# arkworks-rs/groth16

Hardware: AMD Instinct MI355X
Metric: R1CS constraints/sec (create_proof, BLS12-381) (higher is better)
Workload: dtype u32-limb Montgomery integers (Fr 255-bit, Fq 381-bit); 1 GPU; SYN(k=22) synthetic R1CS, 4194302 constraints, FFT domain 2^22, bls12_381, full create_proof (7 NTTs + 4 G1 MSMs + 1 G2 MSM), valid proving key generated on the GPU from seeded toxic waste; curve=bls12_381, log2_domain=22, constraints=4194302, key=valid, witness=resident in HBM at entry (--full: value_incl_h2d holds the PCIe-inclusive rates), parallelism=single-gpu

## Files before the change

groth16_amd/csrc/internal.hpp:

```cpp
#pragma once
#include <hip/hip_runtime.h>
#include <atomic>
#include <cstdint>
#include <cstdio>
#include <cstring>
#include <string>
#include <vector>
#include "../../include/g16_mi355x.h"
#include "curve.hpp"

namespace g16 {

void set_last_error(const char* what, hipError_t e, const char* file, int line);

#define G16_HIP_TRY(expr)                                                     \
    do {                                                                      \
        hipError_t e__ = (expr);                                              \
        if (e__ != hipSuccess) {                                              \
            ::g16::set_last_error(#expr, e__, __FILE__, __LINE__);            \
            return e__ == hipErrorOutOfMemory ? G16_ERR_OOM : G16_ERR_HIP;    \
        }                                                                     \
    } while (0)

#define G16_TRY(expr)                  \
// ... 73 lines not shown
                                    const typename C::Fr* cst, hipStream_t st);
template <class C> int scale_by_table(typename C::Fr* data, const typename C::Fr* table, size_t n, hipStream_t st);
template <class C> int gen_power_table(typename C::Fr* out, size_t n, const typename C::Fr& base, const typename C::Fr& scale, bool r30_form,
                                       hipStream_t st);

template <class C>
struct DeviceCircuit {
    typedef typename C::Fr Fr;
    uint64_t num_inputs = 0, num_constraints = 0, num_variables = 0;
    uint64_t* row_ptr[3] = {nullptr, nullptr, nullptr};
    uint32_t* col[3] = {nullptr, nullptr, nullptr};
    Fr* val[3] = {nullptr, nullptr, nullptr};
    uint64_t nnz[3] = {0, 0, 0};
    Domain<C>* dom = nullptr;
    static constexpr int Z_CHUNKS = 8;
    uint64_t need_col[Z_CHUNKS] = {};
};
struct ZUpload {
    const void* host = nullptr;
    hipStream_t copy_stream = nullptr;
    hipEvent_t landed[8] = {};
    int pieces = 0;
};
template <class C> int mark_unit_coefficients(DeviceCircuit<C>* ck, hipStream_t st);
template <class C> int witness_map_device(const DeviceCircuit<C>* ck, const typename C::Fr* d_z, typename C::Fr* d_h, Arena& arena,
                                          hipStream_t st, EventTimer* ntt_timers = nullptr, ZUpload* up = nullptr);

template <class C>
struct DistWm {
    typedef typename C::Fr Fr;
    int rank = 0, world = 1, log_world = 0;
    size_t M = 0, blk = 0;
    Domain<C>* dom_m = nullptr;
    Fr* tw1 = nullptr;
    Fr* sc_mid = nullptr;
    Fr* tw2 = nullptr;
    Fr* sc_out = nullptr;
    Fr wn_fwd[8], wn_inv[8];
    Fr zinv;
};
template <class C> int dwm_create(const DeviceCircuit<C>* ck, int rank, int world, hipStream_t st, DistWm<C>** out);
template <class C> void dwm_destroy(DistWm<C>* d);
template <class C> int dwm_stage(const DeviceCircuit<C>* ck, const DistWm<C>* dw, int stage, const typename C::Fr* d_z,
                                 typename C::Fr* const work[3], typename C::Fr* const recv[3], typename C::Fr* h_local, hipStream_t st);

struct MsmPlan {
    int c = 0;
    int W = 0;
    int groups = 0;
    bool merged = false;
    uint32_t B = 0;
    uint32_t Lmax = 0;
    int affine_levels = 0;
    uint32_t chunk = 0;
    uint32_t K[10];
    int shard_n = 1, shard_r = 0;
    uint32_t buckets() const { return B * (uint32_t)groups; }
    uint32_t G = 8;
    uint32_t chunk_buckets() const { return B >= G ? G : B; }
    uint32_t chunks() const { return B / chunk_buckets(); }
    int chunk_bits() const { int k = 0; while ((1u << k) < chunks()) ++k; return k; }
    int planes() const { return 2 + chunk_bits(); }
    int outputs() const { return groups * planes(); }
};
static constexpr int MSM_MAX_OUTPUTS = 256;
static constexpr int MSM_MERGED_MIN_C = 9, MSM_MERGED_MAX_C = 20;
static constexpr uint64_t MSM_MERGED_MAX_N = (uint64_t)1 << 26;
int make_msm_plan(uint64_t n, int scalar_bits, const uint32_t* modulus_words, int mod_nwords, int merged_c, MsmPlan* plan, int shard_n = 1,
                  int shard_r = 0);
int msm_window_override();
int merged_window_bits(uint64_t n, int scalar_bits, const uint32_t* modulus_words, int mod_nwords);
int msm_plan_windows(int c, int scalar_bits, const uint32_t* modulus_words, int mod_nwords);

struct ScalarSort {
    MsmPlan plan;
    uint64_t n = 0;
    uint32_t* sorted = nullptr;
    uint32_t* offsets = nullptr;
    uint32_t* task_off = nullptr;
    uint32_t* heavy = nullptr;
    uint32_t max_tasks = 0;
    uint32_t max_segments = 0;
    uint64_t max_sorted = 0;
};
template <class C> int sort_scalars(const typename C::Fr* d_scalars, uint64_t n, int merged_c, Arena& arena, hipStream_t st, ScalarSort* out,
                                    int shard_n = 1, int shard_r = 0);

template <class F>
struct MsmBuffers {
    void* partials = nullptr;
    void* chunk_out = nullptr;
    XYZZ<F>* window_sums = nullptr;
};
template <class F> int msm_bucket_pass(const Affine<F>* d_bases, int64_t shift, uint64_t base_count, const ScalarSort& ss, Arena& arena,
                                       hipStream_t st, MsmBuffers<F>* out, EventTimer* bucket_timer);
template <class F>
struct PassJob {
    const Affine<F>* bases;
    int64_t shift;
    uint64_t base_count;
    const ScalarSort* ss;
    MsmBuffers<F>* out;
};
template <class F> int msm_bucket_pass_batch(const PassJob<F>* jobs, int n, Arena& arena, hipStream_t st, EventTimer* bucket_timer);
template <class F> int msm_reduce(const MsmBuffers<F>& buf, const ScalarSort& ss, hipStream_t st);
template <class F> int msm_reduce_batch(const MsmBuffers<F>* const* bufs, const ScalarSort* const* sorts, int n, hipStream_t st, bool heavy_done);
template <class F> int msm_heavy_reduce(const MsmBuffers<F>& buf, const ScalarSort& ss, hipStream_t st);
template <class F> int msm_heavy_reduce_batch(const MsmBuffers<F>* const* bufs, const ScalarSort* const* sorts, int n, hipStream_t st);
template <class F> int convert_bases(Affine<F>* d_bases, uint64_t n, hipStream_t st);
template <class F> XYZZ<F> fold_windows(const XYZZ<F>* window_sums, const MsmPlan& plan);
template <class F> int build_window_tables(const Affine<F>* d_src, uint64_t n, int c, int W, Affine<F>* d_table, hipStream_t st, void* park = nullptr);
template <class F> size_t window_table_park_bytes(uint64_t n, int W);

template <class C>
int generate_parameters_device(hipStream_t st, Arena& arena, const g16_csr_view abc[3], uint64_t ni, uint64_t nc, uint64_t nv,
                               const g16_toxic_waste* tw, const uint64_t* g1_gen, const uint64_t* g2_gen, const g16_params_view* out);
template <class C>
int qap_evaluations_host(const g16_csr_view abc[3], uint64_t ni, uint64_t nc, uint64_t nv, const uint64_t* t, uint64_t* a_out, uint64_t* b_out,
                         uint64_t* c_out, uint64_t* zt_out);

int serialize_points(int curve, int g2, int compressed, const uint64_t* points, uint64_t n, uint8_t* out);
int deserialize_points(int curve, int g2, int compressed, const uint8_t* in, uint64_t n, int validate, uint64_t* points_out);
uint64_t serialized_point_size(int curve, int g2, int compressed);

int mad_rate_device(hipStream_t st, double* mad_per_s);
template <class C> int synth_bases_device(int g2, uint64_t seed, uint64_t first, uint64_t n, void* out_dev, hipStream_t st);

}
```

groth16_amd/csrc/msm.hip:

```cpp
#include "internal.hpp"
#include "msm_common.hpp"
#include "fp30.hpp"
#include "batch_affine.hpp"
#include "window_tables.hpp"
#include <algorithm>
#include <cstdlib>

namespace g16 {

static constexpr int SORT_THREADS = 1024;
static constexpr int ACC_THREADS = 64;
static constexpr int RED_THREADS = 64;
static constexpr int WIN_THREADS = 256;
#ifndef G16_REDUCE_G
#define G16_REDUCE_G 8
#endif
static constexpr uint32_t REDUCE_G = G16_REDUCE_G;

struct PlanDev {
    int c, W;
    uint32_t B;
    uint32_t K[10];
    uint32_t shard_n, shard_r, shard_magic;
};
// ... 34 lines not shown
    uint32_t* hist = reinterpret_cast<uint32_t*>(smem);
    const int w = blockIdx.y;
    for (uint32_t b = threadIdx.x; b < B; b += SORT_THREADS) hist[b] = 0;
    __syncthreads();
    const uint64_t lo = (uint64_t)blockIdx.x * chunk, hi = min(n, lo + chunk);
    const uint16_t* plane = planes + (uint64_t)w * n;
    for (uint64_t p = lo + threadIdx.x; p < hi; p += SORT_THREADS) {
        uint32_t bucket, neg;
        if (digit_to_bucket(plane[p], c, &bucket, &neg)) atomicAdd(&hist[bucket], 1u);
    }
    __syncthreads();
    uint32_t* out = counts + (uint64_t)w * B;
    for (uint32_t b = threadIdx.x; b < B; b += SORT_THREADS) {
        const uint32_t v = hist[b];
        if (v) atomicAdd(&out[b], v);
    }
}

static constexpr int CLASS_THREADS = 256;
static constexpr int MAX_CLASSES = 64;
static constexpr uint32_t SORT_CLASS_LOG = 13;
static constexpr int SORT_M_THREADS = 256;

template <class Fr>
__device__ __forceinline__ void biased_scalar(const Fr& sc, const PlanDev& plan, uint32_t (*sw)[CLASS_THREADS]) {
    uint32_t s[Fr::N];
    sc.to_canonical(s);
    uint64_t carry = 0;
    G16_UNROLL for (int k = 0; k < 10; ++k) {
        carry += (uint64_t)(k < Fr::N ? s[k] : 0u) + plan.K[k];
        sw[k][threadIdx.x] = (uint32_t)carry;
        carry >>= 32;
    }
    sw[10][threadIdx.x] = 0;
}
__device__ __forceinline__ uint32_t window_of(const uint32_t (*sw)[CLASS_THREADS], int w, int c) {
    const int bit = w * c, word = bit >> 5, sh = bit & 31;
    const uint64_t two = (uint64_t)sw[word][threadIdx.x] | ((uint64_t)sw[word + 1][threadIdx.x] << 32);
    return (uint32_t)(two >> sh) & ((1u << c) - 1u);
}

template <class Fr>
__global__ __launch_bounds__(CLASS_THREADS) void class_count_kernel(const Fr* __restrict__ scalars, uint64_t n, PlanDev plan, uint32_t blog,
                                                                    uint32_t Q, uint32_t* __restrict__ block_counts) {
    __shared__ uint32_t sw[MSM_SWORDS][CLASS_THREADS];
    __shared__ uint32_t cnt[MAX_CLASSES];
    if (threadIdx.x < MAX_CLASSES) cnt[threadIdx.x] = 0;
    __syncthreads();
    const uint64_t i = (uint64_t)blockIdx.x * CLASS_THREADS + threadIdx.x;
    if (i < n) {
        biased_scalar(scalars[i], plan, sw);
        for (int w = 0; w < plan.W; ++w) {
            uint32_t key, neg;
            if (digit_to_bucket(window_of(sw, w, plan.c), plan.c, &key, &neg) && shard_local_key(plan, &key)) atomicAdd(&cnt[key >> blog], 1u);
        }
    }
    __syncthreads();
    if (threadIdx.x < Q) block_counts[(uint64_t)threadIdx.x * gridDim.x + blockIdx.x] = cnt[threadIdx.x];
}

template <class Fr>
__global__ __launch_bounds__(CLASS_THREADS) void class_partition_kernel(const Fr* __restrict__ scalars, uint64_t n, PlanDev plan, uint32_t blog,
                                                                        uint32_t Q, const uint32_t* __restrict__ block_off,
                                                                        uint16_t* __restrict__ ent_key, uint32_t* __restrict__ ent_tag) {
    __shared__ uint32_t sw[MSM_SWORDS][CLASS_THREADS];
    __shared__ uint32_t cur[MAX_CLASSES];
    if (threadIdx.x < Q) cur[threadIdx.x] = block_off[(uint64_t)threadIdx.x * gridDim.x + blockIdx.x];
    __syncthreads();
    const uint64_t i = (uint64_t)blockIdx.x * CLASS_THREADS + threadIdx.x;
    if (i >= n) return;
    biased_scalar(scalars[i], plan, sw);
    for (int w = 0; w < plan.W; ++w) {
        uint32_t key, neg;
        if (digit_to_bucket(window_of(sw, w, plan.c), plan.c, &key, &neg) && shard_local_key(plan, &key)) {
            const uint32_t pos = atomicAdd(&cur[key >> blog], 1u);
            ent_key[pos] = (uint16_t)((key & ((1u << blog) - 1u)) | (neg << 15));
            ent_tag[pos] = (uint32_t)i | ((uint32_t)w << 26);
        }
    }
}

static __global__ __launch_bounds__(SORT_M_THREADS) void bucket_count_merged_kernel(const uint16_t* __restrict__ ent_key,
                                                                           const uint32_t* __restrict__ class_off, uint32_t nb, uint32_t B,
                                                                           uint32_t* __restrict__ wg_counts) {
    extern __shared__ __attribute__((aligned(16))) unsigned char smem[];
    uint32_t* hist = reinterpret_cast<uint32_t*>(smem);
    const uint32_t q = blockIdx.y;
    const uint32_t lo = class_off[(uint64_t)q * nb], hi = class_off[(uint64_t)(q + 1) * nb];
    for (uint32_t b = threadIdx.x; b < B; b += SORT_M_THREADS) hist[b] = 0;
    __syncthreads();
    for (uint64_t p = (uint64_t)lo + blockIdx.x * SORT_M_THREADS + threadIdx.x; p < hi; p += (uint64_t)gridDim.x * SORT_M_THREADS)
        atomicAdd(&hist[ent_key[p] & 0x7fffu], 1u);
    __syncthreads();
    uint32_t* out = wg_counts + ((uint64_t)q * gridDim.x + blockIdx.x) * B;
    for (uint32_t b = threadIdx.x; b < B; b += SORT_M_THREADS) out[b] = hist[b];
}

static __global__ __launch_bounds__(256) void bucket_wg_scan_kernel(uint32_t* __restrict__ wg_counts, uint32_t G, uint32_t B, uint32_t M,
                                                                    uint32_t* __restrict__ counts) {
    const uint32_t i = blockIdx.x * 256 + threadIdx.x;
    if (i >= M) return;
    const uint32_t q = i / B, b = i - q * B;
    uint32_t* col = wg_counts + (uint64_t)q * G * B + b;
    uint32_t run = 0;
    for (uint32_t x = 0; x < G; ++x) {
        const uint32_t v = col[(uint64_t)x * B];
        col[(uint64_t)x * B] = run;
        run += v;
    }
    counts[i] = run;
}

static __global__ __launch_bounds__(SORT_M_THREADS) void bucket_scatter_merged_kernel(const uint16_t* __restrict__ ent_key,
                                                                             const uint32_t* __restrict__ ent_tag,
                                                                             const uint32_t* __restrict__ class_off, uint32_t nb, uint32_t B,
                                                                             const uint32_t* __restrict__ offsets,
                                                                             const uint32_t* __restrict__ wg_counts, uint32_t* __restrict__ sorted) {
    extern __shared__ __attribute__((aligned(16))) unsigned char smem[];
    uint32_t* hist = reinterpret_cast<uint32_t*>(smem);
    const uint32_t q = blockIdx.y;
    const uint32_t lo = class_off[(uint64_t)q * nb], hi = class_off[(uint64_t)(q + 1) * nb];
    if ((uint64_t)lo + (uint64_t)blockIdx.x * SORT_M_THREADS >= hi) return;
    const uint64_t qb = (uint64_t)q * B;
    const uint32_t* mine = wg_counts + ((uint64_t)q * gridDim.x + blockIdx.x) * B;
    for (uint32_t b = threadIdx.x; b < B; b += SORT_M_THREADS) hist[b] = offsets[qb + b] + mine[b];
    __syncthreads();
    const uint64_t first = (uint64_t)lo + blockIdx.x * SORT_M_THREADS + threadIdx.x, step = (uint64_t)gridDim.x * SORT_M_THREADS;
    for (uint64_t p = first; p < hi; p += step) {
        const uint32_t d = ent_key[p];
        const uint32_t pos = atomicAdd(&hist[d & 0x7fffu], 1u);
        sorted[pos] = ent_tag[p] | ((d >> 15) << 31);
    }
}

static constexpr int SCAN_THREADS = 256;
static constexpr int SCAN_PER_THREAD = 8;
static constexpr int SCAN_TILE = SCAN_THREADS * SCAN_PER_THREAD;
static constexpr uint32_t HEAVY_PARTS = 16;

__device__ __forceinline__ uint32_t block_exclusive(uint32_t v, uint32_t* sh, uint32_t* total) {
    const uint32_t tid = threadIdx.x;
    sh[tid] = v;
    __syncthreads();
    for (uint32_t d = 1; d < SCAN_THREADS; d <<= 1) {
        const uint32_t add = tid >= d ? sh[tid - d] : 0u;
        __syncthreads();
        sh[tid] += add;
        __syncthreads();
    }
    const uint32_t incl = sh[tid];
    *total = sh[SCAN_THREADS - 1];
    __syncthreads();
    return incl - v;
}

static __global__ __launch_bounds__(SCAN_THREADS) void scan_block_sums_kernel(const uint32_t* __restrict__ vals, uint32_t M, uint32_t pad,
                                                                       uint32_t* __restrict__ block_sums) {
    __shared__ uint32_t sa[SCAN_THREADS];
    const uint32_t base = blockIdx.x * SCAN_TILE + threadIdx.x * SCAN_PER_THREAD;
    uint32_t sum = 0, tot;
    G16_UNROLL for (int j = 0; j < SCAN_PER_THREAD; ++j) sum += (base + j < M) ? ((vals[base + j] + pad) & ~pad) : 0u;
    (void)block_exclusive(sum, sa, &tot);
    if (threadIdx.x == 0) block_sums[blockIdx.x] = tot;
}

static __global__ __launch_bounds__(SCAN_THREADS) void scan_block_offsets_kernel(uint32_t* __restrict__ block_sums, uint32_t nblocks, uint32_t M,
                                                                          uint32_t* __restrict__ prefix) {
    __shared__ uint32_t sa[SCAN_THREADS];
    uint32_t carry = 0;
    for (uint32_t base = 0; base < nblocks; base += SCAN_THREADS) {
        const uint32_t i = base + threadIdx.x;
        const uint32_t a = i < nblocks ? block_sums[i] : 0u;
        uint32_t tot;
        const uint32_t ea = block_exclusive(a, sa, &tot);
        if (i < nblocks) block_sums[i] = carry + ea;
        carry += tot;
    }
    if (threadIdx.x == 0) prefix[M] = carry;
}

static __global__ __launch_bounds__(SCAN_THREADS) void scan_write_kernel(const uint32_t* __restrict__ vals, uint32_t M, uint32_t pad,
                                                                  const uint32_t* __restrict__ block_base, uint32_t* __restrict__ prefix) {
    __shared__ uint32_t sa[SCAN_THREADS];
    const uint32_t base = blockIdx.x * SCAN_TILE + threadIdx.x * SCAN_PER_THREAD;
    uint32_t cv[SCAN_PER_THREAD], sum = 0, tot;
    G16_UNROLL for (int j = 0; j < SCAN_PER_THREAD; ++j) { cv[j] = (base + j < M) ? ((vals[base + j] + pad) & ~pad) : 0u; sum += cv[j]; }
    uint32_t a = block_base[blockIdx.x] + block_exclusive(sum, sa, &tot);
    G16_UNROLL for (int j = 0; j < SCAN_PER_THREAD; ++j) {
        if (base + j < M) { prefix[base + j] = a; a += cv[j]; }
    }
}

static __global__ void bucket_slots_kernel(const uint32_t* __restrict__ offsets, uint32_t M, uint32_t off_shift, uint32_t lseg,
                                    uint32_t* __restrict__ nparts, uint32_t* __restrict__ heavy ) {
    const uint32_t b = blockIdx.x * blockDim.x + threadIdx.x;
    if (b >= M) return;
    const uint32_t lo = offsets[b] >> off_shift, hi = offsets[b + 1] >> off_shift;
    const uint32_t np = hi > lo ? ((hi - 1) / lseg - lo / lseg + 1u) : 0u;
    nparts[b] = np;
    if (np > HEAVY_PARTS) heavy[1 + atomicAdd(&heavy[0], 1u)] = b;
}

static __global__ __launch_bounds__(SORT_THREADS) void bucket_scatter_kernel(const uint16_t* __restrict__ planes, uint64_t n, uint32_t chunk,
                                                                      int c, uint32_t B, const uint32_t* __restrict__ offsets,
                                                                      uint32_t* __restrict__ cursor, uint32_t* __restrict__ sorted) {
    extern __shared__ __attribute__((aligned(16))) unsigned char smem[];
    uint32_t* hist = reinterpret_cast<uint32_t*>(smem);
    const int w = blockIdx.y;
    for (uint32_t b = threadIdx.x; b < B; b += SORT_THREADS) hist[b] = 0;
    __syncthreads();
    const uint64_t lo = (uint64_t)blockIdx.x * chunk, hi = min(n, lo + chunk);
    const uint16_t* plane = planes + (uint64_t)w * n;
    for (uint64_t p = lo + threadIdx.x; p < hi; p += SORT_THREADS) {
        uint32_t bucket, neg;
        if (digit_to_bucket(plane[p], c, &bucket, &neg)) atomicAdd(&hist[bucket], 1u);
    }
    __syncthreads();
    const uint64_t wb = (uint64_t)w * B;
    for (uint32_t b = threadIdx.x; b < B; b += SORT_THREADS) {
        const uint32_t v = hist[b];
        if (v) hist[b] = offsets[wb + b] + atomicAdd(&cursor[wb + b], v);
    }
    __syncthreads();
    for (uint64_t p = lo + threadIdx.x; p < hi; p += SORT_THREADS) {
        uint32_t bucket, neg;
        if (digit_to_bucket(plane[p], c, &bucket, &neg)) {
            const uint32_t pos = atomicAdd(&hist[bucket], 1u);
            sorted[pos] = (uint32_t)p | (neg << 31);
        }
    }
}

template <class F30>
struct LdsAccStore {
    static constexpr int NL = F30::PREFIX_LIMBS;
    static constexpr int QUADS = NL / 4, TAIL = NL % 4;
    static constexpr int WORDS_PER_VALUE = NL * ACC_THREADS;
    uint32_t* quad;
    uint32_t* tail;
    __device__ __forceinline__ F30 ld(int v) const {
        asm volatile("" ::: "memory");
        uint32_t w[NL];
        const uint32_t* q = quad + v * WORDS_PER_VALUE;
        G16_UNROLL for (int g = 0; g < QUADS; ++g) {
            const uint4 t = *reinterpret_cast<const uint4*>(q + g * 4 * ACC_THREADS);
            w[4 * g] = t.x; w[4 * g + 1] = t.y; w[4 * g + 2] = t.z; w[4 * g + 3] = t.w;
        }
        const uint32_t* r = tail + v * WORDS_PER_VALUE;
        G16_UNROLL for (int i = 0; i < TAIL; ++i) w[4 * QUADS + i] = r[i * ACC_THREADS];
        return F30::from_limbs(w);
    }
    __device__ __forceinline__ void st(int v, const F30& a) const {
        uint32_t w[NL];
        a.get_limbs(w);
        uint32_t* q = quad + v * WORDS_PER_VALUE;
        G16_UNROLL for (int g = 0; g < QUADS; ++g)
            *reinterpret_cast<uint4*>(q + g * 4 * ACC_THREADS) = make_uint4(w[4 * g], w[4 * g + 1], w[4 * g + 2], w[4 * g + 3]);
        uint32_t* r = tail + v * WORDS_PER_VALUE;
        G16_UNROLL for (int i = 0; i < TAIL; ++i) r[i * ACC_THREADS] = w[4 * QUADS + i];
        asm volatile("" ::: "memory");
    }
};

template <class F30>
struct RawAccStore {
    AccRaw<typename F30::Raw>* p;
    __device__ __forceinline__ F30 ld(int k) const {
        asm volatile("" ::: "memory");
        if constexpr (F30::LANES_PER_TASK == 1) {
            static_assert(sizeof(F30) == sizeof(typename F30::Raw), "one-lane fields share the raw layout");
            return reinterpret_cast<const F30*>(p)[k];
        } else {
            typedef typename F30::B B30;
            return F30{reinterpret_cast<const B30*>(p)[2 * k + (F30::lane_hi() ? 1 : 0)]};
        }
    }
    __device__ __forceinline__ void st(int k, const F30& a) const {
        if constexpr (F30::LANES_PER_TASK == 1) {
            reinterpret_cast<F30*>(p)[k] = a;
        } else {
            typedef typename F30::B B30;
            reinterpret_cast<B30*>(p)[2 * k + (F30::lane_hi() ? 1 : 0)] = a.c;
        }
// ... 406 lines not shown
    uint64_t chunk = (n + nchunks - 1) / nchunks;
    chunk = (chunk + 1023) / 1024 * 1024;
    if (chunk < 1024) chunk = 1024;
    plan->chunk = (uint32_t)chunk;
    return G16_OK;
}

#endif

static int ilog2(uint32_t v) { int l = 0; while ((1u << l) < v) ++l; return l; }

template <class C>
int sort_scalars(const typename C::Fr* d_scalars, uint64_t n, int merged_c, Arena& arena, hipStream_t st, ScalarSort* out, int shard_n,
                 int shard_r) {
    typedef typename C::Fr Fr;
    if (n >= ((uint64_t)1 << 31)) return G16_ERR_BAD_LENGTH;
    uint32_t modw[Fr::N];
    for (int i = 0; i < Fr::N; ++i) modw[i] = Fr::Params::mod(i);
    MsmPlan plan;
    G16_TRY(make_msm_plan(n, Fr::Params::BITS, modw, Fr::N, merged_c, &plan, shard_n, shard_r));
    out->plan = plan;
    out->n = n;
    const uint32_t M = plan.buckets();
    const uint64_t nw = n * (uint64_t)plan.W;
    if (nw >= ((uint64_t)1 << 32)) return G16_ERR_BAD_LENGTH;
    uint16_t* planes = nullptr;
    uint32_t* ent_tag = nullptr;
    uint32_t *class_cnt = nullptr, *class_off = nullptr;
    uint32_t *counts = nullptr, *cursor = nullptr, *nparts = nullptr, *block_sums = nullptr;
    uint32_t sort_class_log = SORT_CLASS_LOG;
    if (const char* e = getenv("G16_SORT_CLASS_LOG")) {
        const int v = atoi(e);
        if (v >= 8 && v <= 15) sort_class_log = (uint32_t)v;
    }
    const uint32_t slog = plan.merged ? std::min<uint32_t>(sort_class_log, (uint32_t)ilog2(plan.B)) : 0u;
    const uint32_t Bs = plan.merged ? 1u << slog : plan.B;
    const uint32_t nb = (uint32_t)((n + CLASS_THREADS - 1) / CLASS_THREADS), Q = plan.merged ? M >> slog : (uint32_t)plan.groups;
    G16_TRY(arena.alloc_n(nw ? nw : 1, &planes));
    if (plan.merged) {
        if (Q > MAX_CLASSES) return G16_ERR_INTERNAL;
        G16_TRY(arena.alloc_n(nw ? nw : 1, &ent_tag));
        G16_TRY(arena.alloc_n((size_t)Q * nb + 1, &class_cnt));
        G16_TRY(arena.alloc_n((size_t)Q * nb + 1, &class_off));
    }
    G16_TRY(arena.alloc_n((size_t)3 * M + 1, &counts));
    cursor = counts + M;
    out->heavy = counts + 2 * (size_t)M;
    G16_TRY(arena.alloc_n((size_t)M + 1, &out->offsets));
    G16_TRY(arena.alloc_n((size_t)M + 1, &out->task_off));
    G16_TRY(arena.alloc_n((size_t)M, &nparts));
    const int R = plan.affine_levels;
    const uint32_t pad = (1u << R) - 1u;
    const uint64_t max_sorted = nw + (uint64_t)M * pad;
    if (max_sorted >= ((uint64_t)1 << 32)) return G16_ERR_BAD_LENGTH;
    out->max_sorted = max_sorted;
    G16_TRY(arena.alloc_n(max_sorted ? max_sorted : 1, &out->sorted));
    if (R) G16_HIP_TRY(hipMemsetAsync(out->sorted, 0xff, max_sorted * sizeof(uint32_t), st));
    const uint64_t walked = R ? (max_sorted >> R) : nw;
    out->max_segments = (uint32_t)((walked + plan.Lmax - 1) / plan.Lmax);
    out->max_tasks = out->max_segments + M;
    G16_HIP_TRY(hipMemsetAsync(counts, 0, ((size_t)2 * M + 1) * sizeof(uint32_t), st));
    PlanDev pd;
    pd.c = plan.c; pd.W = plan.W; pd.B = plan.B;
    for (int k = 0; k < 10; ++k) pd.K[k] = plan.K[k];
    pd.shard_n = (uint32_t)plan.shard_n;
    pd.shard_r = (uint32_t)plan.shard_r;
    pd.shard_magic = plan.shard_n > 1 ? (uint32_t)((((uint64_t)1 << 32) + (uint64_t)plan.shard_n - 1) / (uint64_t)plan.shard_n) : 0u;
    const size_t lds = (size_t)Bs * sizeof(uint32_t);
    static PerDeviceOnce attr_once;
    std::atomic<bool>& attr_set = attr_once.flag();
    if (!attr_set) {
        G16_HIP_TRY(hipFuncSetAttribute(reinterpret_cast<const void*>(&bucket_count_kernel), hipFuncAttributeMaxDynamicSharedMemorySize,
                                        128 * 1024));
        G16_HIP_TRY(hipFuncSetAttribute(reinterpret_cast<const void*>(&bucket_scatter_kernel), hipFuncAttributeMaxDynamicSharedMemorySize,
                                        128 * 1024));
        G16_HIP_TRY(hipFuncSetAttribute(reinterpret_cast<const void*>(&bucket_count_merged_kernel),
                                        hipFuncAttributeMaxDynamicSharedMemorySize, 128 * 1024));
        G16_HIP_TRY(hipFuncSetAttribute(reinterpret_cast<const void*>(&bucket_scatter_merged_kernel),
                                        hipFuncAttributeMaxDynamicSharedMemorySize, 128 * 1024));
        attr_set = true;
    }
    const unsigned nchunks = (unsigned)((n + plan.chunk - 1) / plan.chunk);
    const uint32_t blog = plan.merged ? slog : (uint32_t)ilog2(plan.B);
    const uint32_t max_scan = std::max(M, plan.merged ? Q * nb : 0u);
    G16_TRY(arena.alloc_n((size_t)(max_scan + SCAN_TILE - 1) / SCAN_TILE, &block_sums));
    auto prefix_scan = [&](const uint32_t* vals, uint32_t* prefix, uint32_t count, uint32_t padmask = 0) -> int {
        const uint32_t nblocks = (count + SCAN_TILE - 1) / SCAN_TILE;
        hipLaunchKernelGGL(scan_block_sums_kernel, dim3(nblocks), dim3(SCAN_THREADS), 0, st, vals, count, padmask, block_sums);
        G16_LAUNCH_CHECK();
        hipLaunchKernelGGL(scan_block_offsets_kernel, dim3(1), dim3(SCAN_THREADS), 0, st, block_sums, nblocks, count, prefix);
        G16_LAUNCH_CHECK();
        hipLaunchKernelGGL(scan_write_kernel, dim3(nblocks), dim3(SCAN_THREADS), 0, st, vals, count, padmask, block_sums, prefix);
        G16_LAUNCH_CHECK();
        return G16_OK;
    };
    unsigned gx = std::max(1u, std::min(std::min(4096u / Q, 256u), (unsigned)((nw + SORT_M_THREADS - 1) / SORT_M_THREADS)));
    if (const char* e = getenv("G16_SORT_GX")) {
        const int v = atoi(e);
        if (v >= 1 && v <= 4096) gx = (unsigned)v;
    }
    uint32_t* wg_counts = nullptr;
    if (plan.merged) G16_TRY(arena.alloc_n((size_t)Q * gx * Bs, &wg_counts));
    if (n) {
        if (plan.merged) {
            hipLaunchKernelGGL((class_count_kernel<Fr>), dim3(nb), dim3(CLASS_THREADS), 0, st, d_scalars, n, pd, blog, Q, class_cnt);
            G16_LAUNCH_CHECK();
            G16_TRY(prefix_scan(class_cnt, class_off, Q * nb));
            hipLaunchKernelGGL((class_partition_kernel<Fr>), dim3(nb), dim3(CLASS_THREADS), 0, st, d_scalars, n, pd, blog, Q, class_off, planes,
                               ent_tag);
            G16_LAUNCH_CHECK();
            hipLaunchKernelGGL(bucket_count_merged_kernel, dim3(gx, Q), dim3(SORT_M_THREADS), lds, st, planes, class_off, nb, Bs, wg_counts);
            G16_LAUNCH_CHECK();
            hipLaunchKernelGGL(bucket_wg_scan_kernel, dim3((M + 255) / 256), dim3(256), 0, st, wg_counts, gx, Bs, M, counts);
        } else {
            hipLaunchKernelGGL((digits_kernel<Fr>), dim3((unsigned)((n + 255) / 256)), dim3(256), 0, st, d_scalars, n, pd, planes);
            G16_LAUNCH_CHECK();
            hipLaunchKernelGGL(bucket_count_kernel, dim3(nchunks, plan.W), dim3(SORT_THREADS), lds, st, planes, n, plan.chunk, plan.c, plan.B,
                               counts);
        }
        G16_LAUNCH_CHECK();
    }
    G16_TRY(prefix_scan(counts, out->offsets, M, pad));
    hipLaunchKernelGGL(bucket_slots_kernel, dim3((M + 255) / 256), dim3(256), 0, st, out->offsets, M, (uint32_t)R, plan.Lmax, nparts,
                       out->heavy);
    G16_LAUNCH_CHECK();
    G16_TRY(prefix_scan(nparts, out->task_off, M));
    if (n) {
        if (plan.merged)
            hipLaunchKernelGGL(bucket_scatter_merged_kernel, dim3(gx, Q), dim3(SORT_M_THREADS), lds, st, planes, ent_tag, class_off, nb, Bs,
                               out->offsets, wg_counts, out->sorted);
        else
            hipLaunchKernelGGL(bucket_scatter_kernel, dim3(nchunks, plan.W), dim3(SORT_THREADS), lds, st, planes, n, plan.chunk, plan.c, plan.B,
                               out->offsets, cursor, out->sorted);
        G16_LAUNCH_CHECK();
    }
    return G16_OK;
}

template <class F>
static int alloc_msm_buffers(const ScalarSort& ss, Arena& arena, MsmBuffers<F>* out) {
    typedef AccRaw<typename Lazy30<F>::type::Raw> Raw;
    const MsmPlan& plan = ss.plan;
    const uint32_t cpw = plan.B / plan.chunk_buckets();
    Raw *partials = nullptr, *chunk_out = nullptr;
    G16_TRY(arena.alloc_n((size_t)ss.max_tasks ? ss.max_tasks : 1, &partials));
    G16_TRY(arena.alloc_n((size_t)cpw * plan.groups * 2, &chunk_out));
    G16_TRY(arena.alloc_n((size_t)plan.outputs(), &out->window_sums));
    out->partials = partials;
    out->chunk_out = chunk_out;
    return G16_OK;
}

template <class F>
int msm_bucket_pass(const Affine<F>* d_bases, int64_t shift, uint64_t base_count, const ScalarSort& ss, Arena& arena, hipStream_t st,
                    MsmBuffers<F>* out, EventTimer* bucket_timer) {
    typedef typename Lazy30<F>::type F30;
    typedef AccRaw<typename Lazy30<F>::type::Raw> Raw;
    const MsmPlan& plan = ss.plan;
    const uint32_t M = plan.buckets();
    const int R = plan.affine_levels;
    if (!R || !ss.max_sorted) {
        const PassJob<F> job{d_bases, shift, base_count, &ss, out};
        return msm_bucket_pass_batch<F>(&job, 1, arena, st, bucket_timer);
    }
    G16_TRY(alloc_msm_buffers<F>(ss, arena, out));
    Raw* partials = static_cast<Raw*>(out->partials);
    Affine<F>* lists[2] = {nullptr, nullptr};
    Word4* prefix = nullptr;
    constexpr uint32_t T = 64 / F30::LANES_PER_TASK;
    constexpr int QUADS = AffineLevel<F30, true>::QUADS;
    auto level_K = [&](int r) -> uint32_t {
        const uint64_t pairs = ss.max_sorted >> (r + 1);
        uint32_t K = 64;
        while (K > 8 && pairs / ((uint64_t)K * T) < 2048) K >>= 1;
        return K;
    };
    auto level_waves = [&](int r) -> uint64_t { return ((ss.max_sorted >> (r + 1)) + (uint64_t)level_K(r) * T - 1) / ((uint64_t)level_K(r) * T); };
    {
        G16_TRY(arena.alloc_n((size_t)(ss.max_sorted >> 1) + 1, &lists[0]));
        if (R > 1) G16_TRY(arena.alloc_n((size_t)(ss.max_sorted >> 2) + 1, &lists[1]));
        size_t recs = 0;
        for (int r = 0; r < R; ++r) recs = std::max(recs, (size_t)(level_waves(r) * level_K(r)) * QUADS * 64);
        G16_TRY(arena.alloc_n(recs ? recs : 1, &prefix));
    }
    if (bucket_timer) G16_TRY(bucket_timer->start(st));
    {
        AffineLevelArgs<F30> a;
        a.sorted = ss.sorted;
        a.total = ss.offsets + M;
        a.prefix = prefix;
        a.shift = shift;
        a.base_count = base_count;
        a.merged = plan.merged ? 1u : 0u;
        for (int r = 0; r < R; ++r) {
            a.in = r == 0 ? d_bases : lists[(r - 1) & 1];
            a.out = lists[r & 1];
            a.level = (uint32_t)r;
            a.K = level_K(r);
            const uint64_t waves = level_waves(r);
            const unsigned blocks = (unsigned)((waves * 64 + AFF_THREADS - 1) / AFF_THREADS);
            if (r == 0) hipLaunchKernelGGL((affine_level_kernel<F30, true>), dim3(blocks), dim3(AFF_THREADS), 0, st, a);
            else hipLaunchKernelGGL((affine_level_kernel<F30, false>), dim3(blocks), dim3(AFF_THREADS), 0, st, a);
            G16_LAUNCH_CHECK();
        }
    }
    if (ss.max_segments) {
        const uint64_t lanes = (uint64_t)ss.max_segments * F30::LANES_PER_TASK;
        const dim3 grid((unsigned)((lanes + ACC_THREADS - 1) / ACC_THREADS));
        PassBatch<F30> b;
        for (int i = 0; i < PASS_BATCH; ++i) {
            b.bases[i] = lists[(R - 1) & 1]; b.shift[i] = 0; b.base_count[i] = 0; b.sorted[i] = nullptr;
            b.offsets[i] = ss.offsets; b.slot_off[i] = ss.task_off; b.partials[i] = partials;
        }
// ... 256 lines not shown
```

groth16_amd/csrc/unit_api.hpp:

```cpp
#pragma once
#include "api_types.hpp"
#include "prover.hpp"

namespace {

template <class C>
struct UnitApi {
    typedef typename C::Fr Fr;
    typedef typename C::Fq Fq;
    typedef typename C::Fq2 Fq2;
    typedef typename C::G1A G1A;
    typedef typename C::G2A G2A;
    typedef typename C::G1X G1X;
    typedef typename C::G2X G2X;
    static constexpr int L = Fq::N / 2;
    static int witness_map_api(g16_ctx* ctx, const g16_circuit* ckh, const uint64_t* z, uint64_t n_assign, int on_device, uint64_t* h_out) {
        const DeviceCircuit<C>* ck = static_cast<const DeviceCircuit<C>*>(ckh->dc);
        if (n_assign != ck->num_variables) return G16_ERR_BAD_LENGTH;
        DrainOnError drain(ctx);
        ctx->reset_arena();
        const Fr* d_z = nullptr;
        G16_TRY(Prover<C>::stage_assignment(ctx, z, n_assign, on_device, &d_z));
        Fr* d_h = nullptr;
        G16_TRY(ctx->arena.alloc_n(ck->dom->n, &d_h));
        G16_TRY((witness_map_device<C>(ck, d_z, d_h, ctx->arena, ctx->stream)));
        G16_HIP_TRY(hipMemcpyAsync(h_out, d_h, ck->dom->n * sizeof(Fr), hipMemcpyDeviceToHost, ctx->stream));
        G16_HIP_TRY(hipStreamSynchronize(ctx->stream));
        drain.dismiss();
        return G16_OK;
    }

    static int dwm_stage_api(g16_ctx* ctx, const g16_circuit* ckh, const void* dwp, int stage, const uint64_t* z, uint64_t n_assign, int on_device,
                             uint64_t* const work[3], uint64_t* const recv[3], uint64_t* h_local, bool async) {
        const DeviceCircuit<C>* ck = static_cast<const DeviceCircuit<C>*>(ckh->dc);
        const DistWm<C>* dw = static_cast<const DistWm<C>*>(dwp);
        DrainOnError drain(ctx);
        const Fr* d_z = nullptr;
        if (stage == 0) {
            if (!z || n_assign != ck->num_variables) return G16_ERR_BAD_LENGTH;
            if (async) {
                if (!on_device) return G16_ERR_BAD_ARG;
                d_z = reinterpret_cast<const Fr*>(z);
            } else {
                ctx->reset_arena();
                G16_TRY(Prover<C>::stage_assignment(ctx, z, n_assign, on_device, &d_z));
            }
        }
        Fr* w[3] = {reinterpret_cast<Fr*>(work[0]), reinterpret_cast<Fr*>(work[1]), reinterpret_cast<Fr*>(work[2])};
        Fr* rv[3] = {reinterpret_cast<Fr*>(recv[0]), reinterpret_cast<Fr*>(recv[1]), reinterpret_cast<Fr*>(recv[2])};
        G16_TRY((dwm_stage<C>(ck, dw, stage, d_z, w, rv, reinterpret_cast<Fr*>(h_local), async ? ctx->stream_wm : ctx->stream)));
        if (!async) G16_HIP_TRY(hipStreamSynchronize(ctx->stream));
        drain.dismiss();
        return G16_OK;
    }

    template <class F>
    static int msm_api(g16_ctx* ctx, const uint64_t* bases, const uint64_t* scalars, uint64_t n, uint64_t* out_affine, int shard_n = 1,
                       int shard_r = 0) {
        typedef Affine<F> A;
        typedef XYZZ<F> X;
        hipStream_t st = ctx->stream;
        DrainOnError drain(ctx);
        ctx->reset_arena();
        A* d_b = nullptr;
        Fr* d_s = nullptr;
        G16_TRY(ctx->arena.alloc_n(n ? n : 1, &d_b));
        G16_TRY(ctx->arena.alloc_n(n ? n : 1, &d_s));
        if (n) {
            G16_HIP_TRY(hipMemcpyAsync(d_b, bases, n * sizeof(A), hipMemcpyHostToDevice, st));
            G16_HIP_TRY(hipMemcpyAsync(d_s, scalars, n * sizeof(Fr), hipMemcpyHostToDevice, st));
        }
        int merged_c = 0;
        const char* e = getenv("G16_MSM_API_PRECOMP");
        uint32_t modw[Fr::N];
        for (int i = 0; i < Fr::N; ++i) modw[i] = Fr::Params::mod(i);
        if (((e && atoi(e) != 0) || shard_n > 1) && n) merged_c = merged_window_bits(n, Fr::Params::BITS, modw, Fr::N);
        if (shard_n > 1 && n && !merged_c) return G16_ERR_BAD_ARG;
        if (shard_n > 1 && !n) { memset(out_affine, 0, sizeof(A)); drain.dismiss(); return G16_OK; }
        if (merged_c) {
            const int W = msm_plan_windows(merged_c, Fr::Params::BITS, modw, Fr::N);
            A* d_t = nullptr;
            G16_TRY(ctx->arena.alloc_n((size_t)n * W, &d_t));
            G16_TRY((build_window_tables<F>(d_b, n, merged_c, W, d_t, st)));
            d_b = d_t;
        } else {
            G16_TRY((convert_bases<F>(d_b, n, st)));
        }
        ScalarSort ss;
        G16_TRY((sort_scalars<C>(d_s, n, merged_c, ctx->arena, st, &ss, shard_n, shard_r)));
        MsmBuffers<F> buf;
        G16_TRY((msm_bucket_pass<F>(d_b, 0, n, ss, ctx->arena, st, &buf, &ctx->t_bucket[0])));
        G16_TRY((msm_reduce<F>(buf, ss, st)));
        std::vector<X> hws(ss.plan.outputs());
        G16_HIP_TRY(hipMemcpyAsync(hws.data(), buf.window_sums, sizeof(X) * ss.plan.outputs(), hipMemcpyDeviceToHost, st));
        G16_HIP_TRY(hipStreamSynchronize(st));
        drain.dismiss();
        const A res = fold_windows<F>(hws.data(), ss.plan).to_affine();
        memcpy(out_affine, &res, sizeof(A));
        ctx->tm.bucket_pass_ms = ctx->t_bucket[0].ms();
        ctx->tm.bucket_ms[0] = ctx->tm.bucket_pass_ms;
        ctx->tm.window_bits = ss.plan.c;
        ctx->tm.windows = ss.plan.W;
        return G16_OK;
    }

    static int ntt_api(g16_ctx* ctx, uint64_t* data, int log_n, int inverse, int coset) {
        if (log_n < 0 || log_n > 30) return G16_ERR_DEGREE_TOO_LARGE;
        hipStream_t st = ctx->stream;
        Domain<C>* dom = nullptr;
        G16_TRY((domain_create<C>(log_n, st, &dom)));
        const size_t n = dom->n;
        ctx->reset_arena();
        Fr *d_a = nullptr, *d_o = nullptr;
        int rc = G16_OK;
        auto body = [&]() -> int {
            G16_TRY(ctx->arena.alloc_n(n, &d_a));
            G16_TRY(ctx->arena.alloc_n(n, &d_o));
            G16_HIP_TRY(hipMemcpyAsync(d_a, data, n * sizeof(Fr), hipMemcpyHostToDevice, st));
            if (!inverse) {
                if (coset) {
                    G16_TRY((domain_ensure_gpow<C>(dom, st)));
                    G16_TRY((scale_by_table<C>(d_a, dom->g_pow, n, st)));
                }
                G16_TRY((ntt_dif<C>(dom, d_a, false, st)));
                G16_TRY((bitrev_scale<C>(dom, d_o, d_a, nullptr, nullptr, st)));
            } else {
                G16_TRY((ntt_dif<C>(dom, d_a, true, st)));
                if (coset) G16_TRY((bitrev_scale<C>(dom, d_o, d_a, dom->s2, nullptr, st)));
                else G16_TRY((bitrev_scale<C>(dom, d_o, d_a, nullptr, &dom->n_inv, st)));
            }
            G16_HIP_TRY(hipMemcpyAsync(data, d_o, n * sizeof(Fr), hipMemcpyDeviceToHost, st));
            G16_HIP_TRY(hipStreamSynchronize(st));
            return G16_OK;
        };
        rc = body();
        domain_destroy<C>(dom);
        return rc;
    }

    template <class F>
    static int field_op(int op, const uint64_t* a, const uint64_t* b, uint64_t* out) {
        F x = load_pod<F>(a), y = b ? load_pod<F>(b) : F::zero(), r;
        switch (op) {
            case 0: r = x + y; break;
            case 1: r = x - y; break;
            case 2: r = x * y; break;
            case 3: r = x.inverse(); break;
            case 4: x.to_canonical(r.v); break;
            case 5: r = F::from_canonical(x.v); break;
            default: return G16_ERR_BAD_ARG;
        }
        memcpy(out, &r, sizeof(F));
        return G16_OK;
    }
    template <class F>
    static int group_op(int op, const uint64_t* p_, const uint64_t* q_, uint64_t* out) {
        typedef Affine<F> A;
        typedef XYZZ<F> X;
        const A p = load_pod<A>(p_);
        X acc = X::from_affine(p);
        if (op == 0) {
            acc.add_affine(load_pod<A>(q_));
        } else if (op == 1) {
            uint32_t k[8];
            memcpy(k, q_, 32);
            acc = acc.mul_bits(k, 256);
        } else if (op == 2) {
            X q = X::from_affine(load_pod<A>(q_));
            X p2 = acc.dbl(), q2 = q.dbl();
            p2.add(q2);
            X np = acc.neg();
            p2.add(np);
            X nq = q.neg();
            p2.add(nq);
            acc = p2;
        } else {
            return G16_ERR_BAD_ARG;
        }
        const A r = acc.to_affine();
// ... 78 lines not shown
```

Before: 65.56 million constraints/s.

## Add two-level local bucket sort for merged MSM scalar sorting

The merged-window scalar sort now partitions each class into 128-bucket sub-ranges first. Sub-ranges small enough are then sorted inside one workgroup using LDS staging, which gives coalesced writes. Classes with an oversized sub-range fall back to the existing global count/scan/scatter path, controlled by per-class flags. The intent is to replace the scattered global-atomic histogram and scatter with cache-friendly local sorting. The cost is extra passes and extra key/tag buffers.

```diff
diff --git a/groth16_amd/csrc/internal.hpp b/groth16_amd/csrc/internal.hpp
--- a/groth16_amd/csrc/internal.hpp
+++ b/groth16_amd/csrc/internal.hpp
@@ -179,6 +179,7 @@
     uint32_t max_tasks = 0;
     uint32_t max_segments = 0;
     uint64_t max_sorted = 0;
+    uint32_t* stats = nullptr;
 };
 template <class C> int sort_scalars(const typename C::Fr* d_scalars, uint64_t n, int merged_c, Arena& arena, hipStream_t st, ScalarSort* out,
                                     int shard_n = 1, int shard_r = 0);
diff --git a/groth16_amd/csrc/msm.hip b/groth16_amd/csrc/msm.hip
--- a/groth16_amd/csrc/msm.hip
+++ b/groth16_amd/csrc/msm.hip
@@ -140,10 +140,11 @@
 
 static __global__ __launch_bounds__(SORT_M_THREADS) void bucket_count_merged_kernel(const uint16_t* __restrict__ ent_key,
                                                                            const uint32_t* __restrict__ class_off, uint32_t nb, uint32_t B,
-                                                                           uint32_t* __restrict__ wg_counts) {
+                                                                           const uint32_t* __restrict__ flag, uint32_t* __restrict__ wg_counts) {
     extern __shared__ __attribute__((aligned(16))) unsigned char smem[];
     uint32_t* hist = reinterpret_cast<uint32_t*>(smem);
     const uint32_t q = blockIdx.y;
+    if (flag && !flag[q]) return;
     const uint32_t lo = class_off[(uint64_t)q * nb], hi = class_off[(uint64_t)(q + 1) * nb];
     for (uint32_t b = threadIdx.x; b < B; b += SORT_M_THREADS) hist[b] = 0;
     __syncthreads();
@@ -155,10 +156,11 @@
 }
 
 static __global__ __launch_bounds__(256) void bucket_wg_scan_kernel(uint32_t* __restrict__ wg_counts, uint32_t G, uint32_t B, uint32_t M,
-                                                                    uint32_t* __restrict__ counts) {
+                                                                    const uint32_t* __restrict__ flag, uint32_t* __restrict__ counts) {
     const uint32_t i = blockIdx.x * 256 + threadIdx.x;
     if (i >= M) return;
     const uint32_t q = i / B, b = i - q * B;
+    if (flag && !flag[q]) return;
     uint32_t* col = wg_counts + (uint64_t)q * G * B + b;
     uint32_t run = 0;
     for (uint32_t x = 0; x < G; ++x) {
@@ -172,11 +174,12 @@
 static __global__ __launch_bounds__(SORT_M_THREADS) void bucket_scatter_merged_kernel(const uint16_t* __restrict__ ent_key,
                                                                              const uint32_t* __restrict__ ent_tag,
                                                                              const uint32_t* __restrict__ class_off, uint32_t nb, uint32_t B,
-                                                                             const uint32_t* __restrict__ offsets,
+                                                                             const uint32_t* __restrict__ offsets, const uint32_t* __restrict__ flag,
                                                                              const uint32_t* __restrict__ wg_counts, uint32_t* __restrict__ sorted) {
     extern __shared__ __attribute__((aligned(16))) unsigned char smem[];
     uint32_t* hist = reinterpret_cast<uint32_t*>(smem);
     const uint32_t q = blockIdx.y;
+    if (flag && !flag[q]) return;
     const uint32_t lo = class_off[(uint64_t)q * nb], hi = class_off[(uint64_t)(q + 1) * nb];
     if ((uint64_t)lo + (uint64_t)blockIdx.x * SORT_M_THREADS >= hi) return;
     const uint64_t qb = (uint64_t)q * B;
@@ -257,6 +260,172 @@
     const uint32_t np = hi > lo ? ((hi - 1) / lseg - lo / lseg + 1u) : 0u;
     nparts[b] = np;
     if (np > HEAVY_PARTS) heavy[1 + atomicAdd(&heavy[0], 1u)] = b;
+}
+
+static constexpr uint32_t SUB_LOG = 7;
+static constexpr uint32_t SUB_BUCKETS = 1u << SUB_LOG;
+static constexpr int SUB_THREADS = 256;
+static constexpr uint32_t SUB_TILE = 2048;
+static constexpr uint32_t LOCAL_TILE = 1024;
+static constexpr uint32_t LOCAL_MAX = 1u << 16;
+
+struct SubTile { uint32_t q, lo, hi, cidx, cstride; };
+
+__device__ __forceinline__ bool sub_tile_of(const uint32_t* __restrict__ class_off, uint32_t nb, uint32_t Q, uint32_t subs, uint32_t slot,
+                                            uint32_t* sh, SubTile* t) {
+    if (threadIdx.x == 0) sh[0] = 0xffffffffu;
+    __syncthreads();
+    if (threadIdx.x < Q) {
+        const uint32_t q = threadIdx.x, a = class_off[(uint64_t)q * nb], b = class_off[(uint64_t)(q + 1) * nb];
+        const uint32_t tb = a / SUB_TILE + q, nt = (b - a + SUB_TILE - 1) / SUB_TILE;
+        if (slot >= tb && slot - tb < nt) {
+            const uint32_t j = slot - tb;
+            sh[0] = q;
+            sh[1] = a + j * SUB_TILE;
+            sh[2] = (uint32_t)min((uint64_t)b, (uint64_t)a + (uint64_t)(j + 1) * SUB_TILE);
+            sh[3] = subs * tb + j;
+            sh[4] = nt;
+        }
+    }
+    __syncthreads();
+    t->q = sh[0]; t->lo = sh[1]; t->hi = sh[2]; t->cidx = sh[3]; t->cstride = sh[4];
+    return t->q != 0xffffffffu;
+}
+
+static __global__ __launch_bounds__(SUB_THREADS) void sub_count_kernel(const uint16_t* __restrict__ ent_key, const uint32_t* __restrict__ class_off,
+                                                                       uint32_t nb, uint32_t Q, uint32_t sublog, uint32_t subs,
+                                                                       uint32_t* __restrict__ tile_counts) {
+    __shared__ uint32_t sh[5];
+    __shared__ uint32_t cnt[MAX_CLASSES];
+    if (threadIdx.x < MAX_CLASSES) cnt[threadIdx.x] = 0;
+    SubTile t;
+    if (!sub_tile_of(class_off, nb, Q, subs, blockIdx.x, sh, &t)) return;
+    for (uint32_t p = t.lo + threadIdx.x; p < t.hi; p += SUB_THREADS) atomicAdd(&cnt[(ent_key[p] & 0x7fffu) >> sublog], 1u);
+    __syncthreads();
+    if (threadIdx.x < subs) tile_counts[t.cidx + threadIdx.x * t.cstride] = cnt[threadIdx.x];
+}
+
+static __global__ __launch_bounds__(SUB_THREADS) void sub_partition_kernel(const uint16_t* __restrict__ ent_key, const uint32_t* __restrict__ ent_tag,
+                                                                           const uint32_t* __restrict__ class_off, uint32_t nb, uint32_t Q,
+                                                                           uint32_t sublog, uint32_t subs, const uint32_t* __restrict__ tile_pos,
+                                                                           uint16_t* __restrict__ out_key, uint32_t* __restrict__ out_tag) {
+    __shared__ uint32_t sh[5];
+    __shared__ uint32_t cur[MAX_CLASSES];
+    SubTile t;
+    if (!sub_tile_of(class_off, nb, Q, subs, blockIdx.x, sh, &t)) return;
+    if (threadIdx.x < subs) cur[threadIdx.x] = tile_pos[t.cidx + threadIdx.x * t.cstride];
+    __syncthreads();
+    for (uint32_t p = t.lo + threadIdx.x; p < t.hi; p += SUB_THREADS) {
+        const uint32_t d = ent_key[p];
+        const uint32_t pos = atomicAdd(&cur[(d & 0x7fffu) >> sublog], 1u);
+        out_key[pos] = (uint16_t)d;
+        out_tag[pos] = ent_tag[p];
+    }
+}
+
+static __global__ __launch_bounds__(64) void sub_flag_kernel(const uint32_t* __restrict__ class_off, uint32_t nb, uint32_t Q, uint32_t subs,
+                                                             const uint32_t* __restrict__ tile_pos, uint32_t local_max,
+                                                             uint32_t* __restrict__ sub_start, uint32_t* __restrict__ flag,
+                                                             uint32_t* __restrict__ stats, uint32_t* __restrict__ total_out) {
+    const uint32_t q = blockIdx.x, sub = threadIdx.x;
+    const uint32_t a = class_off[(uint64_t)q * nb], b = class_off[(uint64_t)(q + 1) * nb];
+    const uint32_t tb = a / SUB_TILE + q, nt = (b - a + SUB_TILE - 1) / SUB_TILE;
+    uint32_t s = b;
+    if (sub < subs) s = nt ? tile_pos[subs * tb + sub * nt] : a;
+    uint32_t next = __shfl_down(s, 1, 64);
+    if (sub + 1 >= subs) next = b;
+    const bool big = sub < subs && next - s > local_max;
+    const bool any = __any(big ? 1 : 0) != 0;
+    if (sub < subs) sub_start[q * subs + sub] = s;
+    if (sub == 0) {
+        flag[q] = any ? 1u : 0u;
+        atomicAdd(&stats[any ? 0 : 1], 1u);
+        if (q == Q - 1) { sub_start[Q * subs] = b; *total_out = b; }
+    }
+}
+
+__device__ __forceinline__ uint32_t wave_inclusive(uint32_t x) {
+    const uint32_t lane = threadIdx.x & 63u;
+    G16_UNROLL for (uint32_t d = 1; d < 64; d <<= 1) {
+        const uint32_t y = __shfl_up(x, d, 64);
+        if (lane >= d) x += y;
+    }
+    return x;
+}
+__device__ __forceinline__ void sub_scan128(const uint32_t* a, uint32_t base, uint32_t* out) {
+    static_assert(SUB_BUCKETS == 128, "two values per lane of one wave");
+    if (threadIdx.x < 64) {
+        const uint32_t a0 = a[2 * threadIdx.x], a1 = a[2 * threadIdx.x + 1];
+        const uint32_t ex = base + wave_inclusive(a0 + a1) - (a0 + a1);
+        out[2 * threadIdx.x] = ex;
+        out[2 * threadIdx.x + 1] = ex + a0;
+    }
+}
+
+static __global__ __launch_bounds__(SUB_THREADS) void sub_local_sort_kernel(const uint16_t* __restrict__ ent_key, const uint32_t* __restrict__ ent_tag,
+                                                                            const uint32_t* __restrict__ sub_start, const uint32_t* __restrict__ flag,
+                                                                            uint32_t subs, uint32_t sublog, uint32_t* __restrict__ offsets,
+                                                                            uint32_t* __restrict__ sorted) {
+    __shared__ uint32_t cur[SUB_BUCKETS], tcnt[SUB_BUCKETS], tstart[SUB_BUCKETS], stage[LOCAL_TILE];
+    __shared__ uint8_t sbkt[LOCAL_TILE];
+    constexpr int PER = LOCAL_TILE / SUB_THREADS;
+    const uint32_t sc = blockIdx.x;
+    if (flag[sc / subs]) return;
+    const uint32_t s0 = sub_start[sc], s1 = sub_start[sc + 1], nbk = 1u << sublog, mask = nbk - 1u;
+    if (threadIdx.x < SUB_BUCKETS) { tcnt[threadIdx.x] = 0; tstart[threadIdx.x] = 0; }
+    __syncthreads();
+    for (uint32_t p = s0 + threadIdx.x; p < s1; p += SUB_THREADS) atomicAdd(&tstart[ent_key[p] & mask], 1u);
+    __syncthreads();
+    sub_scan128(tstart, s0, cur);
+    __syncthreads();
+    if (threadIdx.x < nbk) offsets[sc * nbk + threadIdx.x] = cur[threadIdx.x];
+    for (uint32_t base = s0; base < s1; base += LOCAL_TILE) {
+        uint32_t bk[PER], val[PER], rank[PER];
+        G16_UNROLL for (int j = 0; j < PER; ++j) {
+            const uint32_t p = base + j * SUB_THREADS + threadIdx.x;
+            bk[j] = 0xffffffffu;
+            if (p < s1) {
+                const uint32_t d = ent_key[p];
+                bk[j] = d & mask;
+                val[j] = ent_tag[p] | ((d >> 15) << 31);
+                rank[j] = atomicAdd(&tcnt[bk[j]], 1u);
+            }
+        }
+        __syncthreads();
+        sub_scan128(tcnt, 0, tstart);
+        __syncthreads();
+        G16_UNROLL for (int j = 0; j < PER; ++j) {
+            if (bk[j] != 0xffffffffu) {
+                const uint32_t slot = tstart[bk[j]] + rank[j];
+                stage[slot] = val[j];
+                sbkt[slot] = (uint8_t)bk[j];
+            }
+        }
+        __syncthreads();
+        const uint32_t nin = min(LOCAL_TILE, s1 - base);
+        for (uint32_t i = threadIdx.x; i < nin; i += SUB_THREADS) {
+            const uint32_t b = sbkt[i];
+            sorted[cur[b] + (i - tstart[b])] = stage[i];
+        }
+        __syncthreads();
+        if (threadIdx.x < SUB_BUCKETS) { cur[threadIdx.x] += tcnt[threadIdx.x]; tcnt[threadIdx.x] = 0; }
+        __syncthreads();
+    }
+}
+
+static __global__ __launch_bounds__(SCAN_THREADS) void class_bucket_offsets_kernel(const uint32_t* __restrict__ counts,
+                                                                                  const uint32_t* __restrict__ class_off, uint32_t nb, uint32_t B,
+                                                                                  const uint32_t* __restrict__ flag, uint32_t* __restrict__ offsets) {
+    __shared__ uint32_t sa[SCAN_THREADS];
+    const uint32_t q = blockIdx.x;
+    if (!flag[q]) return;
+    const uint32_t per = (B + SCAN_THREADS - 1) / SCAN_THREADS, first = threadIdx.x * per;
+    const uint32_t* in = counts + (uint64_t)q * B;
+    uint32_t sum = 0, tot;
+    for (uint32_t j = first; j < min(B, first + per); ++j) sum += in[j];
+    uint32_t a = class_off[(uint64_t)q * nb] + block_exclusive(sum, sa, &tot);
+    uint32_t* out = offsets + (uint64_t)q * B;
+    for (uint32_t j = first; j < min(B, first + per); ++j) { out[j] = a; a += in[j]; }
 }
 
 static __global__ __launch_bounds__(SORT_THREADS) void bucket_scatter_kernel(const uint16_t* __restrict__ planes, uint64_t n, uint32_t chunk,
@@ -829,7 +998,27 @@
     }
     const unsigned nchunks = (unsigned)((n + plan.chunk - 1) / plan.chunk);
     const uint32_t blog = plan.merged ? slog : (uint32_t)ilog2(plan.B);
-    const uint32_t max_scan = std::max(M, plan.merged ? Q * nb : 0u);
+    bool local = plan.merged && R == 0;
+    if (const char* e = getenv("G16_SORT_LOCAL")) local = local && atoi(e) != 0;
+    const uint32_t sublog = std::min<uint32_t>(SUB_LOG, slog), subs = Bs >> sublog, NS = Q * subs;
+    const uint32_t ntiles = (uint32_t)(nw / SUB_TILE) + Q + 1;
+    if (subs > MAX_CLASSES) local = false;
+    if (local && (uint64_t)subs * ntiles >= ((uint64_t)1 << 32)) return G16_ERR_BAD_LENGTH;
+    uint16_t* key2 = nullptr;
+    uint32_t *tag2 = nullptr, *tile_cnt = nullptr, *tile_pos = nullptr, *sub_start = nullptr, *flag = nullptr;
+    out->stats = nullptr;
+    if (local) {
+        G16_TRY(arena.alloc_n(nw ? nw : 1, &key2));
+        G16_TRY(arena.alloc_n(nw ? nw : 1, &tag2));
+        G16_TRY(arena.alloc_n((size_t)subs * ntiles + 1, &tile_cnt));
+        G16_TRY(arena.alloc_n((size_t)subs * ntiles + 1, &tile_pos));
+        G16_TRY(arena.alloc_n((size_t)NS + 1, &sub_start));
+        G16_TRY(arena.alloc_n((size_t)Q + 2, &flag));
+        out->stats = flag + Q;
+        G16_HIP_TRY(hipMemsetAsync(tile_cnt, 0, ((size_t)subs * ntiles + 1) * sizeof(uint32_t), st));
+        G16_HIP_TRY(hipMemsetAsync(flag, 0, ((size_t)Q + 2) * sizeof(uint32_t), st));
+    }
+    const uint32_t max_scan = std::max(std::max(M, plan.merged ? Q * nb : 0u), local ? subs * ntiles : 0u);
     G16_TRY(arena.alloc_n((size_t)(max_scan + SCAN_TILE - 1) / SCAN_TILE, &block_sums));
     auto prefix_scan = [&](const uint32_t* vals, uint32_t* prefix, uint32_t count, uint32_t padmask = 0) -> int {
         const uint32_t nblocks = (count + SCAN_TILE - 1) / SCAN_TILE;
@@ -856,9 +1045,32 @@
             hipLaunchKernelGGL((class_partition_kernel<Fr>), dim3(nb), dim3(CLASS_THREADS), 0, st, d_scalars, n, pd, blog, Q, class_off, planes,
                                ent_tag);
             G16_LAUNCH_CHECK();
-            hipLaunchKernelGGL(bucket_count_merged_kernel, dim3(gx, Q), dim3(SORT_M_THREADS), lds, st, planes, class_off, nb, Bs, wg_counts);
-            G16_LAUNCH_CHECK();
-            hipLaunchKernelGGL(bucket_wg_scan_kernel, dim3((M + 255) / 256), dim3(256), 0, st, wg_counts, gx, Bs, M, counts);
+            if (local) {
+                hipLaunchKernelGGL(sub_count_kernel, dim3(ntiles), dim3(SUB_THREADS), 0, st, planes, class_off, nb, Q, sublog, subs, tile_cnt);
+                G16_LAUNCH_CHECK();
+                G16_TRY(prefix_scan(tile_cnt, tile_pos, subs * ntiles));
+                hipLaunchKernelGGL(sub_partition_kernel, dim3(ntiles), dim3(SUB_THREADS), 0, st, planes, ent_tag, class_off, nb, Q, sublog, subs,
+                                   tile_pos, key2, tag2);
+                G16_LAUNCH_CHECK();
+                hipLaunchKernelGGL(sub_flag_kernel, dim3(Q), dim3(64), 0, st, class_off, nb, Q, subs, tile_pos, LOCAL_MAX, sub_start, flag,
+                                   out->stats, out->offsets + M);
+                G16_LAUNCH_CHECK();
+                hipLaunchKernelGGL(sub_local_sort_kernel, dim3(NS), dim3(SUB_THREADS), 0, st, key2, tag2, sub_start, flag, subs, sublog,
+                                   out->offsets, out->sorted);
+                G16_LAUNCH_CHECK();
+                hipLaunchKernelGGL(bucket_count_merged_kernel, dim3(gx, Q), dim3(SORT_M_THREADS), lds, st, key2, class_off, nb, Bs, flag, wg_counts);
+                G16_LAUNCH_CHECK();
+                hipLaunchKernelGGL(bucket_wg_scan_kernel, dim3((M + 255) / 256), dim3(256), 0, st, wg_counts, gx, Bs, M, flag, counts);
+                G16_LAUNCH_CHECK();
+                hipLaunchKernelGGL(class_bucket_offsets_kernel, dim3(Q), dim3(SCAN_THREADS), 0, st, counts, class_off, nb, Bs, flag, out->offsets);
+                G16_LAUNCH_CHECK();
+                hipLaunchKernelGGL(bucket_scatter_merged_kernel, dim3(gx, Q), dim3(SORT_M_THREADS), lds, st, key2, tag2, class_off, nb, Bs,
+                                   out->offsets, flag, wg_counts, out->sorted);
+            } else {
+                hipLaunchKernelGGL(bucket_count_merged_kernel, dim3(gx, Q), dim3(SORT_M_THREADS), lds, st, planes, class_off, nb, Bs, nullptr, wg_counts);
+                G16_LAUNCH_CHECK();
+                hipLaunchKernelGGL(bucket_wg_scan_kernel, dim3((M + 255) / 256), dim3(256), 0, st, wg_counts, gx, Bs, M, nullptr, counts);
+            }
         } else {
             hipLaunchKernelGGL((digits_kernel<Fr>), dim3((unsigned)((n + 255) / 256)), dim3(256), 0, st, d_scalars, n, pd, planes);
             G16_LAUNCH_CHECK();
@@ -867,15 +1079,15 @@
         }
         G16_LAUNCH_CHECK();
     }
-    G16_TRY(prefix_scan(counts, out->offsets, M, pad));
+    if (!local || !n) G16_TRY(prefix_scan(counts, out->offsets, M, pad));
     hipLaunchKernelGGL(bucket_slots_kernel, dim3((M + 255) / 256), dim3(256), 0, st, out->offsets, M, (uint32_t)R, plan.Lmax, nparts,
                        out->heavy);
     G16_LAUNCH_CHECK();
     G16_TRY(prefix_scan(nparts, out->task_off, M));
-    if (n) {
+    if (n && !local) {
         if (plan.merged)
             hipLaunchKernelGGL(bucket_scatter_merged_kernel, dim3(gx, Q), dim3(SORT_M_THREADS), lds, st, planes, ent_tag, class_off, nb, Bs,
-                               out->offsets, wg_counts, out->sorted);
+                               out->offsets, nullptr, wg_counts, out->sorted);
         else
             hipLaunchKernelGGL(bucket_scatter_kernel, dim3(nchunks, plan.W), dim3(SORT_THREADS), lds, st, planes, n, plan.chunk, plan.c, plan.B,
                                out->offsets, cursor, out->sorted);
diff --git a/groth16_amd/csrc/unit_api.hpp b/groth16_amd/csrc/unit_api.hpp
--- a/groth16_amd/csrc/unit_api.hpp
+++ b/groth16_amd/csrc/unit_api.hpp
@@ -93,8 +93,11 @@
         G16_TRY((msm_reduce<F>(buf, ss, st)));
         std::vector<X> hws(ss.plan.outputs());
         G16_HIP_TRY(hipMemcpyAsync(hws.data(), buf.window_sums, sizeof(X) * ss.plan.outputs(), hipMemcpyDeviceToHost, st));
+        uint32_t sort_stats[2] = {0, 0};
+        if (ss.stats) G16_HIP_TRY(hipMemcpyAsync(sort_stats, ss.stats, sizeof(sort_stats), hipMemcpyDeviceToHost, st));
         G16_HIP_TRY(hipStreamSynchronize(st));
         drain.dismiss();
+        if (ss.stats && getenv("G16_DEBUG")) fprintf(stderr, "g16 sort classes: matrix %u local %u\n", sort_stats[0], sort_stats[1]);
         const A res = fold_windows<F>(hws.data(), ss.plan).to_affine();
         memcpy(out_affine, &res, sizeof(A));
         ctx->tm.bucket_pass_ms = ctx->t_bucket[0].ms();
```

Result: no change. 65.77 million constraints/s (median of 6 runs) (+0.3%).
